# Sudaraka88/LDWeaver

Measured on NVIDIA B200. Metric: weighted SNP-pair MI/sec, higher is better.
Workload: dtype int8 (tcgen05 kind::i8 with int32 accumulation of 28-bit fixed-point weights; fp32 MI epilogue, fp64 refinement of long-range links)

## Files before the change

### ldweaver_b200/csrc/mi_aux.cuh

```cuda
#pragma once
#include "mi_types.h"

namespace ldw {

__global__ void mi_build_rec_kernel(const uint8_t* __restrict__ codes, int64_t S, const int32_t* __restrict__ slot_snp,
                                    int64_t nslots, const uint8_t* __restrict__ mask, const double* __restrict__ w,
                                    const int32_t* __restrict__ wH, const int32_t* __restrict__ wL, Rec* rec,
                                    int64_t vstride, double* p64 , uint32_t sa, uint32_t sb, uint32_t M) {
  int64_t slot = (int64_t)blockIdx.x * (blockDim.x >> 5) + (threadIdx.x >> 5);
  int lane = threadIdx.x & 31;
  if (slot >= nslots) return;
  int32_t snp = slot_snp[slot];
  if (snp < 0) {
    if (lane < 4) {
      Rec z;
      for (int q = 0; q < 4; q++) { z.T[q] = 0; z.rp[q] = 0.f; z.q[q] = 1.f; }
      z.T4 = 0; z.rp4 = 0.f; z.q4 = 1.f; z.pad = 0;
      rec[lane * vstride + slot] = z;
    }
    return;
  }
  const uint8_t* row = codes + (int64_t)snp * S;
  double p[5] = {0, 0, 0, 0, 0};
  int h[5] = {0, 0, 0, 0, 0}, l[5] = {0, 0, 0, 0, 0};
// ... 21 lines not shown
    for (int a = 0; a < 5; a++) p64[(int64_t)snp * 5 + a] = p[a];
  if (lane < 4) {
    int m = mask[snp];
    uint32_t qt[5] = {0, 0, 0, 0, 0};
    float qr[5] = {0.f, 0.f, 0.f, 0.f, 0.f}, qq[5] = {1.f, 1.f, 1.f, 1.f, 1.f};
    int q = 0;
    for (int a = 0; a < 5; a++) {
      if (m & (1 << a)) {
        qt[q] = ((uint32_t)h[a] << sa) + ((uint32_t)l[a] >> sb) + M * (uint32_t)(lane + 2);
        const double v = p[a] + 0.5 * (double)(lane + 2);
        qr[q] = (float)(1.0 / v);
        qq[q] = (float)v;
        q++;
      }
    }
    Rec z;
    for (int t = 0; t < 4; t++) { z.T[t] = qt[t]; z.rp[t] = qr[t]; z.q[t] = qq[t]; }
    z.T4 = qt[4]; z.rp4 = qr[4]; z.q4 = qq[4]; z.pad = 0;
    rec[lane * vstride + slot] = z;
  }
}

__global__ void mi_pack_operands_kernel(const uint8_t* __restrict__ codes, int64_t S, int64_t Kpad,
                                        const uint32_t* __restrict__ row_info, int64_t nrows, uint8_t* X) {
  int64_t chunks = Kpad / 16;
  int64_t id = (int64_t)blockIdx.x * blockDim.x + threadIdx.x;
  if (id >= nrows * chunks) return;
  int64_t R = id / chunks, ch = id % chunks;
  uint32_t info = row_info[R];
  uint32_t x1[4] = {0, 0, 0, 0};
  if (info != 0xFFFFFFFFu) {
    const uint8_t* row = codes + (int64_t)(info & 0x0FFFFFFF) * S;
    int al = info >> 28;
    int64_t s0 = ch * 16;
#pragma unroll
    for (int k = 0; k < 16; k++) {
      int64_t s = s0 + k;
      uint32_t bit = (s < S && row[s] == al) ? 0xFFu : 0u;
      x1[k >> 2] |= bit << (8 * (k & 3));
    }
  }
  *reinterpret_cast<uint4*>(X + R * Kpad + ch * 16) = make_uint4(x1[0], x1[1], x1[2], x1[3]);
}

struct RefineParams {
  const uint8_t* codes;
  int64_t S;
  const double* w;
  const double* p64;
  const uint8_t* r;
  const uint8_t* mask;
  const int32_t* from_idx;
  const int32_t* to_idx;
  const uint8_t* rfl_arr;
  const uint8_t* rtl_arr;
  int32_t nf, nt;
  int32_t ideal_q;
  double neff;
};

constexpr int REFINE_WARPS = 6;
__device__ __forceinline__ int heaviest_class(const double (&p)[5]) {
  int b = 0;
#pragma unroll
  for (int a = 1; a < 5; a++) b = p[a] > p[b] ? a : b;
// ... 566 lines not shown
```

### ldweaver_b200/csrc/mi_kernel.cuh

```cuda
#pragma once
#include "mi_types.h"
#include "umma.cuh"

namespace ldw {

constexpr int MI_EXP_WARPS = 6;
constexpr int MI_EXP_THREADS = 32 * MI_EXP_WARPS;
constexpr int MI_EPI_WARP0 = 8;
constexpr int MI_EPI_GROUPS = 4;
constexpr int MI_EPI_WARPS = 4 * MI_EPI_GROUPS;
constexpr int MI_EPI_THREADS = 32 * MI_EPI_WARPS;
constexpr int MI_THREADS = 32 * (MI_EPI_WARP0 + MI_EPI_WARPS);
#define LDW_STR2(x) #x
#define LDW_STR(x) LDW_STR2(x)
#define MI_REGS_CTRL 48
#define MI_REGS_EPI 96
static_assert(MI_EPI_WARP0 * 32 * MI_REGS_CTRL + MI_EPI_THREADS * MI_REGS_EPI <= MI_THREADS * ((65536 / MI_THREADS) & ~7), "register budget");
constexpr int MI_MAX_STAGES = 4;
constexpr uint32_t MI_ARR_BYTES = 128 * 128;
constexpr uint32_t MI_STAGE_REGION = 12 * MI_ARR_BYTES;
__host__ __device__ constexpr uint32_t mi_stage_need(int pa, int pb, int njlog2) {
  return (uint32_t)pa * MI_ARR_BYTES + 4u * (uint32_t)pb * (64u << njlog2);
}
__host__ __device__ constexpr int mi_stage_geo(int pa, int pb, int njlog2) {
  return mi_stage_need(pa, pb, njlog2) <= 3 * MI_ARR_BYTES ? 0 : mi_stage_need(pa, pb, njlog2) <= 4 * MI_ARR_BYTES ? 1 : 2;
}
__host__ __device__ constexpr int mi_geo_stages(int geo) { return 4 - geo; }
__host__ __device__ constexpr uint32_t mi_geo_bytes(int geo) { return geo == 0 ? 3 * MI_ARR_BYTES : geo == 1 ? 4 * MI_ARR_BYTES : 6 * MI_ARR_BYTES; }
constexpr uint32_t MI_JREC_BYTES = 128 * sizeof(Rec);
constexpr uint32_t MI_JDYN_BYTES = 128 * sizeof(ColDyn);
constexpr uint32_t MI_IREC_BYTES = 128 * sizeof(Rec);
constexpr uint32_t MI_IDYN_BYTES = 128 * sizeof(RowDyn);
constexpr uint32_t MI_BAR_BYTES = 512;
constexpr uint32_t MI_SMEM_BYTES = MI_STAGE_REGION + 2 * (MI_JREC_BYTES + MI_JDYN_BYTES) + MI_IREC_BYTES + MI_IDYN_BYTES + MI_BAR_BYTES + 1024;
static_assert(MI_SMEM_BYTES <= 232448, "shared memory budget (227 KB opt-in)");

__device__ __forceinline__ float lg2_fast(float x) {
  float y;
  asm("lg2.approx.ftz.f32 %0, %1;" : "=f"(y) : "f"(x));
  return y;
}
__device__ __forceinline__ uint32_t ld_volatile_u32(const uint32_t* p) {
  uint32_t v;
  asm volatile("ld.volatile.global.u32 %0, [%1];" : "=r"(v) : "l"(p));
  return v;
}

__host__ __device__ constexpr int mi_jc(int pa, int pb) {
  return (pa + 1) * (pb + 1) <= 4 ? 8 : (pa + 1) * (pb + 1) <= 9 ? 4 : (pa + 1) * (pb + 1) <= 12 ? 2 : 1;
}
__host__ __device__ constexpr int mi_njlog2(int pa, int pb) {
  return pa * pb == 1 ? 7 : pa * pb == 2 ? 6 : pa * pb <= 4 ? 5 : 4;
}

__device__ __noinline__ void lr_raise_threshold(const ScanParams& p, int lane) {
  constexpr int PER = MI_HIST_BINS / 32;
  uint32_t s = 0;
  for (int k = 0; k < PER; k++) s += ld_volatile_u32(p.hist + lane * PER + k);
  uint32_t suf = s;
#pragma unroll
  for (int o = 1; o < 32; o <<= 1) {
    uint32_t v = __shfl_down_sync(0xffffffffu, suf, o);
    if (lane + o < 32) suf += v;
  }
  unsigned m = __ballot_sync(0xffffffffu, suf >= p.kprime);
  if (m == 0) return;
  int sel = 31 - __clz(m);
  if (lane == sel) {
    uint32_t run = suf - s;
    for (int k = PER - 1; k >= 0; k--) {
      run += ld_volatile_u32(p.hist + lane * PER + k);
      if (run >= p.kprime) {
        atomicMax(p.tcand_bits, (uint32_t)(lane * PER + k) << 19);
        break;
      }
// ... 7 lines not shown
    long long c0 = clock64();
    mbar_wait(bar, parity, tag);
    acc += clock64() - c0;
  } else {
    mbar_wait(bar, parity, tag);
  }
}

struct EpiCtx {
  int q, cg, lane, rank;
  uint32_t tflags;
  uint32_t tmem_base;
  uint32_t jrec_saddr;
  uint32_t jdyn_saddr;
  uint32_t irec_saddr, idyn_saddr;
  uint32_t rempty_saddr;
  uint32_t scr_saddr;
};

__device__ __forceinline__ uint4 lds128(uint32_t saddr) {
  uint4 v;
  asm volatile("ld.shared.v4.u32 {%0, %1, %2, %3}, [%4];" : "=r"(v.x), "=r"(v.y), "=r"(v.z), "=r"(v.w) : "r"(saddr));
  return v;
}

__device__ __forceinline__ uint2 lds64(uint32_t saddr) {
  uint2 v;
  asm volatile("ld.shared.v2.u32 {%0, %1}, [%2];" : "=r"(v.x), "=r"(v.y) : "r"(saddr));
  return v;
}

__device__ __forceinline__ void sts128(uint32_t saddr, uint4 v) {
  asm volatile("st.shared.v4.u32 [%0], {%1, %2, %3, %4};" ::"r"(saddr), "r"(v.x), "r"(v.y), "r"(v.z), "r"(v.w) : "memory");
}

__device__ __forceinline__ float rcp_fast(float x) {
  float y;
  asm("rcp.approx.ftz.f32 %0, %1;" : "=f"(y) : "f"(x));
  return y;
}

template <bool QC>
__device__ __forceinline__ float mi_term(float acc, uint32_t t, float ra, float rb, float dq) {
  const float x = __uint2float_rn(t);
  const float ratio = QC ? x * rcp_fast(fmaf(ra, rb, dq)) : x * (ra * rb);
  return fmaf(x, lg2_fast(ratio), acc);
// ... 281 lines not shown
  switch (pa * 4 + pb - 5) {
    case 0: epi_tile<1, 1, QC, RG>(p, c, rel); break;
    case 1: epi_tile<1, 2, QC, RG>(p, c, rel); break;
    case 2: epi_tile<1, 3, QC, RG>(p, c, rel); break;
    case 3: epi_tile<1, 4, QC, RG>(p, c, rel); break;
    case 4: epi_tile<2, 1, QC, RG>(p, c, rel); break;
    case 5: epi_tile<2, 2, QC, RG>(p, c, rel); break;
    case 6: epi_tile<2, 3, QC, RG>(p, c, rel); break;
    case 7: epi_tile<2, 4, QC, RG>(p, c, rel); break;
    case 8: epi_tile<3, 1, QC, RG>(p, c, rel); break;
    case 9: epi_tile<3, 2, QC, RG>(p, c, rel); break;
    case 10: epi_tile<3, 3, QC, RG>(p, c, rel); break;
    case 11: epi_tile<3, 4, QC, RG>(p, c, rel); break;
    case 12: epi_tile<4, 1, QC, RG>(p, c, rel); break;
    case 13: epi_tile<4, 2, QC, RG>(p, c, rel); break;
    case 14: epi_tile<4, 3, QC, RG>(p, c, rel); break;
    case 15: epi_tile<4, 4, QC, RG>(p, c, rel); break;
    default: break;
  }
}

template <bool DBG>
__global__ void __cluster_dims__(2, 1, 1) __launch_bounds__(MI_THREADS, 1)
mi_scan_kernel(const __grid_constant__ TmapSet tm, const __grid_constant__ ScanParams p) {
  extern __shared__ uint8_t smem_raw[];
  uint8_t* smem = reinterpret_cast<uint8_t*>((reinterpret_cast<uintptr_t>(smem_raw) + 1023) & ~(uintptr_t)1023);
  uint8_t* stage_base = smem;
  Rec* jrec = reinterpret_cast<Rec*>(smem + MI_STAGE_REGION);
  ColDyn* jdyn = reinterpret_cast<ColDyn*>(smem + MI_STAGE_REGION + 2 * MI_JREC_BYTES);
  Rec* irec = reinterpret_cast<Rec*>(smem + MI_STAGE_REGION + 2 * (MI_JREC_BYTES + MI_JDYN_BYTES));
  RowDyn* idyn = reinterpret_cast<RowDyn*>(smem + MI_STAGE_REGION + 2 * (MI_JREC_BYTES + MI_JDYN_BYTES) + MI_IREC_BYTES);
  uint64_t* bars = reinterpret_cast<uint64_t*>(smem + MI_STAGE_REGION + 2 * (MI_JREC_BYTES + MI_JDYN_BYTES) + MI_IREC_BYTES + MI_IDYN_BYTES);
  uint64_t* full = bars;
  uint64_t* empty = bars + 4;
  uint64_t* ready = bars + 8;
  uint64_t* tfull = bars + 12;
  uint64_t* tempty = bars + 14;
  uint64_t* jfull = bars + 16;
  uint64_t* jempty = bars + 18;
  uint64_t* drained = bars + 20;
  uint64_t* rfull = bars + 21;
  uint64_t* rempty = bars + 22;
  uint32_t* tmem_slot = reinterpret_cast<uint32_t*>(bars + 23);
  uint32_t* thdr = reinterpret_cast<uint32_t*>(bars + 24);

  const int warp = threadIdx.x >> 5, lane = threadIdx.x & 31;
  const uint32_t rank = cluster_ctarank();
  if (warp == 0 && lane == 0) {
    tma_prefetch_desc(&tm.a);
    for (int i = 0; i < MI_MAX_STAGES; i++) {
      mbar_init(&full[i], 1); mbar_init(&empty[i], 1); mbar_init(&ready[i], 2 * MI_EXP_WARPS);
    }
    mbar_init(drained, 1);
    mbar_init(rfull, 1); mbar_init(rempty, MI_EPI_WARPS);
    for (int i = 0; i < 2; i++) {
      mbar_init(&tfull[i], 1); mbar_init(&tempty[i], 2 * MI_EPI_WARPS);
      mbar_init(&jfull[i], 1); mbar_init(&jempty[i], MI_EPI_WARPS);
    }
    fence_barrier_init();
  }
  if (warp == 2) tmem_alloc_pair(tmem_slot, 512);
  tc_fence_before();
  cluster_sync_all();
  tc_fence_after();
  const uint32_t tmem_base = *tmem_slot;
  const int tile0 = (int)(blockIdx.x >> 1), tstep = (int)(gridDim.x >> 1);

  if (warp < MI_EPI_WARP0) {
  asm volatile("setmaxnreg.dec.sync.aligned.u32 " LDW_STR(MI_REGS_CTRL) ";");
  if (warp == 0) {
    int st = 0; uint32_t phb = 0; int geo = -1; uint32_t dph = 0;
    int it = 0, rit = 0;
    long long w_jempty = 0, w_empty = 0, t_begin = DBG ? clock64() : 0;
    for (int t = tile0; t < p.n_tiles; t += tstep, it++) {
      const TileDesc td = p.tiles[t];
      const int PA = td.PA, PB = td.PB, NJ = 1 << td.njlog2, NJh = NJ >> 1;
      const int njidx = 7 - td.njlog2;
      const int g = mi_stage_geo(PA, PB, td.njlog2);
      const int nst = mi_geo_stages(g);
      const uint32_t sbytes = mi_geo_bytes(g);
      if (g != geo) {
        if (geo >= 0) { mbar_wait(drained, dph, 12); dph ^= 1; }
        geo = g; st = 0;
      }
      {
        const uint32_t stage_tx = (uint32_t)PA * MI_ARR_BYTES + (uint32_t)(PB * NJh * 128);
        const int a_row = td.a_row0 + (int)rank * 128, b_row = td.b_row0 + (int)rank * NJh;
        for (int kb = 0; kb < p.nkb; kb++) {
          timed_wait<DBG>(&empty[st], ((phb >> st) & 1) ^ 1, 11, w_empty);
          if (elect_one()) {
            uint8_t* sb = stage_base + st * sbytes;
            mbar_arrive_expect_tx(&full[st], stage_tx);
            for (int a = 0; a < PA; a++)
              tma_load_2d(sb + a * MI_ARR_BYTES, &tm.a, &full[st], kb * 128, a_row + a * td.a_pstride);
            uint8_t* sbB = sb + PA * MI_ARR_BYTES;
            for (int b = 0; b < PB; b++)
              tma_load_2d(sbB + b * NJh * 128, &tm.b[njidx], &full[st], kb * 128, b_row + b * td.b_pstride);
          }
          __syncwarp();
          phb ^= 1u << st;
          if (++st == nst) st = 0;
        }
      }
      const int jb = it & 1;
      timed_wait<DBG>(&jempty[jb], ((it >> 1) & 1) ^ 1, 10, w_jempty);
      if (elect_one()) {
        thdr[jb] = (uint32_t)PA | ((uint32_t)PB << 8) | ((uint32_t)td.njlog2 << 16) | ((uint32_t)(rank ? td.flags1 : td.flags) << 24);
        mbar_arrive_expect_tx(&jfull[jb], (uint32_t)NJ * (uint32_t)(sizeof(Rec) + sizeof(ColDyn)));
        bulk_load_1d(jrec + jb * 128, p.rec + (int64_t)(PA + 1 - 2) * p.rec_vstride + td.j_slot0, NJ * sizeof(Rec), &jfull[jb]);
        bulk_load_1d(jdyn + jb * 128, p.coldyn + td.j_dyn0, NJ * sizeof(ColDyn), &jfull[jb]);
      }
      __syncwarp();
      if (!((rank ? td.flags1 : td.flags) & TILE_NULL)) {
        timed_wait<DBG>(rempty, (uint32_t)(rit & 1) ^ 1, 13, w_jempty);
        if (elect_one()) {
          mbar_arrive_expect_tx(rfull, MI_IREC_BYTES + MI_IDYN_BYTES);
          bulk_load_1d(irec, p.rec + (int64_t)(PB + 1 - 2) * p.rec_vstride + td.i_slot0 + (int)rank * 128, MI_IREC_BYTES, rfull);
          bulk_load_1d(idyn, p.rowdyn + td.i_dyn0 + (int)rank * 128, MI_IDYN_BYTES, rfull);
        }
        __syncwarp();
        rit++;
      }
    }
    if (DBG && p.dbg && lane == 0) {
// ... 65 lines not shown
      }
      if (elect_one()) {
        if (sw) umma_commit_pair(drained);
        if (big) {
          umma_commit_pair(&tfull[0]);
          umma_commit_pair(&tfull[1]);
        } else {
          umma_commit_pair(&tfull[as]);
        }
      }
      __syncwarp();
      if (!big) {
        if (++as == 2) { as = 0; aph ^= 1; }
      }
    }
    if (DBG && p.dbg && lane == 0) {
      p.dbg[blockIdx.x * 16 + 3] = (unsigned long long)(clock64() - t_begin);
      p.dbg[blockIdx.x * 16 + 4] = (unsigned long long)w_tempty;
      p.dbg[blockIdx.x * 16 + 5] = (unsigned long long)w_ready;
    }
    }
  } else {
    const int h = (warp - 2) * 32 + lane;
    int st = 0; uint32_t phb = 0; int geo = -1;
    long long w_full = 0, t_begin = DBG ? clock64() : 0;
    for (int t = tile0; t < p.n_tiles; t += tstep) {
      const TileDesc td = p.tiles[t];
      const int PA = td.PA, PB = td.PB, NJh = (1 << td.njlog2) >> 1;
      const int brows = PB * NJh;
      const int g = mi_stage_geo(PA, PB, td.njlog2);
      const int nst = mi_geo_stages(g);
      const uint32_t sbytes = mi_geo_bytes(g);
      if (g != geo) { geo = g; st = 0; }
      for (int kb = 0; kb < p.nkb; kb++) {
        const int cl = h & 7;
        const uint8_t* dg = p.dig + (int64_t)kb * 128 + cl * 16;
        const uint4 g0 = __ldg(reinterpret_cast<const uint4*>(dg));
        const uint4 g1 = __ldg(reinterpret_cast<const uint4*>(dg + p.kpad));
        const uint4 g2 = __ldg(reinterpret_cast<const uint4*>(dg + 2 * p.kpad));
        const uint4 g3 = __ldg(reinterpret_cast<const uint4*>(dg + 3 * p.kpad));
        timed_wait<DBG>(&full[st], (phb >> st) & 1, 40, w_full);
        const uint32_t yb = smem_u32(stage_base + st * sbytes) + (uint32_t)PA * MI_ARR_BYTES;
        const uint32_t slot = (uint32_t)brows * 128u;
        for (int r = h >> 3; r < brows; r += MI_EXP_THREADS / 8) {
          const uint32_t addr = yb + (uint32_t)r * 128u + (uint32_t)((cl ^ (r & 7)) * 16);
          const uint4 y = lds128(addr);
          sts128(addr + slot, make_uint4(y.x & g1.x, y.y & g1.y, y.z & g1.z, y.w & g1.w));
          sts128(addr + 2 * slot, make_uint4(y.x & g2.x, y.y & g2.y, y.z & g2.z, y.w & g2.w));
          sts128(addr + 3 * slot, make_uint4(y.x & g3.x, y.y & g3.y, y.z & g3.z, y.w & g3.w));
          sts128(addr, make_uint4(y.x & g0.x, y.y & g0.y, y.z & g0.z, y.w & g0.w));
        }
        fence_proxy_async_smem();
        __syncwarp();
        if (lane == 0) mbar_arrive_cluster(&ready[st], 0);
        phb ^= 1u << st;
        if (++st == nst) st = 0;
      }
    }
    if (DBG && p.dbg && h == 0) {
      p.dbg[blockIdx.x * 16 + 12] = (unsigned long long)(clock64() - t_begin);
      p.dbg[blockIdx.x * 16 + 13] = (unsigned long long)w_full;
    }
  }
  } else {
    asm volatile("setmaxnreg.inc.sync.aligned.u32 " LDW_STR(MI_REGS_EPI) ";");
    EpiCtx c;
    c.q = warp & 3;
    c.cg = (warp - MI_EPI_WARP0) >> 2;
    c.lane = lane;
    c.rank = (int)rank;
    int as = 0; uint32_t aph = 0;
    int it = 0, rit = 0;
    long long w_jfull = 0, w_tfull = 0, t_begin = DBG ? clock64() : 0;
    c.irec_saddr = smem_u32(irec);
    c.idyn_saddr = smem_u32(idyn);
    c.rempty_saddr = smem_u32(rempty);
    c.scr_saddr = smem_u32(bars + 32) + (uint32_t)(warp - MI_EPI_WARP0) * 4u;
    for (int t = tile0; t < p.n_tiles; t += tstep, it++) {
      const int jb = it & 1;
      timed_wait<DBG>(&jfull[jb], (it >> 1) & 1, 30, w_jfull);
      uint32_t hdr;
      asm volatile("ld.shared.u32 %0, [%1];" : "=r"(hdr) : "r"(smem_u32(&thdr[jb])));
      const int tPA = (int)(hdr & 0xFF), tPB = (int)((hdr >> 8) & 0xFF);
      c.tflags = hdr >> 24;
// ... 58 lines not shown
```

### ldweaver_b200/csrc/mi_scan.cu

```cuda
#include <algorithm>
#include <chrono>
#include <cmath>
#include <cub/cub.cuh>
#include <vector>

#include "../../include/ldw.h"
#include "ctx.h"
#include "hdw.h"
#include "mi_aux.cuh"
#include "mi_kernel.cuh"
#include "mi_scan.h"

using namespace ldw;

namespace {

struct Group {
  int32_t slot0 = 0, nslots = 0, row0 = 0, count = 0;
};

struct DevLinks {
  DevBuf pos1, pos2, c1, c2, len, blk, mi;
  int ensure(int64_t m) {
    size_t b4 = (size_t)(m > 0 ? m : 1) * 4, b8 = (size_t)(m > 0 ? m : 1) * 8;
// ... 56 lines not shown
};

static void scan_ws_free(void* p) { delete static_cast<ScanWS*>(p); }

static ScanWS* get_ws(ldw_ctx* ctx) {
  if (!ctx->scan_ws) {
    ctx->scan_ws = new ScanWS();
    ctx->scan_ws_free = scan_ws_free;
  }
  return static_cast<ScanWS*>(ctx->scan_ws);
}

struct ldw_mi_plan {
  ldw_ctx* ctx = nullptr;
  int64_t n = 0, S = 0, blk = 0, Kpad = 0;
  int nranges = 0;
  std::vector<int32_t> pos, paint;
  std::vector<uint8_t> r, mask;
  std::vector<double> w;
  std::vector<Group> groups;
  std::vector<int32_t> range_slot0;
  std::vector<int32_t> slot_snp;
  int64_t nslots = 0, nrows = 0;
  double neff = 0, scale = 0;
  int32_t neffH = 0, neffL = 0;
  uint32_t sa = 0, sb = 0;
  uint32_t M = 0;
  bool pos_sorted = true;
  DevBuf d_codes, d_w, d_p64, d_rec, d_r, d_mask, d_pos, d_paint, d_ops, d_dig;
  const uint8_t* codes_dev = nullptr;
  TmapSet tm;
  std::vector<BlockResult> results;
  double t_pack_ms = 0;
};

namespace {

int build_plan(ldw_mi_plan* P, const uint8_t* codes, const uint8_t* codes_dev, const double* hdw, const int32_t* pos,
               const int32_t* paint) {
  ldw_ctx* ctx = P->ctx;
  cudaStream_t st = ctx->stream;
  const int64_t n = P->n, S = P->S, blk = P->blk;
  cudaEvent_t e0, e1;
  LDW_CUDA(cudaEventCreate(&e0));
  LDW_CUDA(cudaEventCreate(&e1));
  LDW_CUDA(cudaEventRecord(e0, st));
  const bool dbg_t = getenv("LDW_DBG_TIMING") != nullptr;
  auto bt0 = std::chrono::steady_clock::now();
  auto blap = [&](const char* what) {
    if (!dbg_t) return;
    auto t = std::chrono::steady_clock::now();
    fprintf(stderr, "ldw timing: plan %-22s %8.3f ms\n", what, std::chrono::duration<double, std::milli>(t - bt0).count());
    bt0 = t;
  };
// ... 144 lines not shown
  LDW_TRY(P->d_w.alloc((size_t)S * 8));
  LDW_TRY(d_wH.alloc((size_t)S * 4));
  LDW_TRY(d_wL.alloc((size_t)S * 4));
  LDW_TRY(d_slot_snp.alloc((size_t)std::max<int64_t>(slot, 1) * 4));
  LDW_TRY(d_row_info.alloc(row_info.size() * 4));
  LDW_TRY(P->d_p64.alloc((size_t)n * 5 * 8));
  LDW_TRY(P->d_rec.alloc((size_t)std::max<int64_t>(slot, 1) * 4 * sizeof(Rec)));
  LDW_TRY(P->d_pos.alloc((size_t)n * 4));
  LDW_TRY(P->d_paint.alloc((size_t)n * 4));
  LDW_CUDA(cudaMemcpyAsync(P->d_w.p, hdw, (size_t)S * 8, cudaMemcpyHostToDevice, st));
  LDW_CUDA(cudaMemcpyAsync(d_wH.p, wH.data(), (size_t)S * 4, cudaMemcpyHostToDevice, st));
  LDW_CUDA(cudaMemcpyAsync(d_wL.p, wL.data(), (size_t)S * 4, cudaMemcpyHostToDevice, st));
  LDW_CUDA(cudaMemcpyAsync(d_slot_snp.p, P->slot_snp.data(), (size_t)slot * 4, cudaMemcpyHostToDevice, st));
  LDW_CUDA(cudaMemcpyAsync(d_row_info.p, row_info.data(), row_info.size() * 4, cudaMemcpyHostToDevice, st));
  LDW_CUDA(cudaMemcpyAsync(P->d_pos.p, pos, (size_t)n * 4, cudaMemcpyHostToDevice, st));
  LDW_CUDA(cudaMemcpyAsync(P->d_paint.p, paint, (size_t)n * 4, cudaMemcpyHostToDevice, st));
  {
    int wpb = 8;
    mi_build_rec_kernel<<<(unsigned)((slot + wpb - 1) / wpb), wpb * 32, 0, st>>>(
        P->codes_dev, S, d_slot_snp.as<int32_t>(), slot, P->d_mask.as<uint8_t>(), P->d_w.as<double>(),
        d_wH.as<int32_t>(), d_wL.as<int32_t>(), P->d_rec.as<Rec>(), slot, P->d_p64.as<double>(), P->sa, P->sb, P->M);
    LDW_CUDA(cudaGetLastError());
  }
  size_t op_bytes = (size_t)std::max<int64_t>(row, 128) * P->Kpad;
  LDW_TRY(P->d_ops.alloc(op_bytes));
  LDW_TRY(P->d_dig.alloc(dig.size()));
  LDW_CUDA(cudaMemcpyAsync(P->d_dig.p, dig.data(), dig.size(), cudaMemcpyHostToDevice, st));
  {
    int64_t total = row * (P->Kpad / 16);
    if (total > 0) {
      mi_pack_operands_kernel<<<(unsigned)((total + 255) / 256), 256, 0, st>>>(P->codes_dev, S, P->Kpad,
                                                                               d_row_info.as<uint32_t>(), row,
                                                                               P->d_ops.as<uint8_t>());
      LDW_CUDA(cudaGetLastError());
    }
  }
  uint64_t trows = (uint64_t)std::max<int64_t>(row, 128);
  LDW_TRY(make_tmap_u8_sw128(&P->tm.a, P->d_ops.p, trows, (uint64_t)P->Kpad, 128));
  for (int j = 0; j < 4; j++) LDW_TRY(make_tmap_u8_sw128(&P->tm.b[j], P->d_ops.p, trows, (uint64_t)P->Kpad, 64u >> j));
  {
    ScanWS* W = get_ws(ctx);
    if (!W->events_ready) {
      for (auto& b : W->ring) {
        LDW_CUDA(cudaEventCreateWithFlags(&b.done, cudaEventDisableTiming));
        LDW_CUDA(cudaEventCreateWithFlags(&b.done2, cudaEventDisableTiming));
        LDW_CUDA(cudaEventCreateWithFlags(&b.uploaded, cudaEventDisableTiming));
      }
      for (auto& l : W->lr) {
        LDW_CUDA(cudaEventCreateWithFlags(&l.scan_done, cudaEventDisableTiming));
        LDW_CUDA(cudaEventCreateWithFlags(&l.sel_done, cudaEventDisableTiming));
      }
      W->events_ready = true;
    }
  }
  LDW_CUDA(cudaEventRecord(e1, st));
  LDW_CUDA(cudaStreamSynchronize(st));
  blap("records + pack + tmaps");
  float ms = 0;
  cudaEventElapsedTime(&ms, e0, e1);
  P->t_pack_ms = ms;
  cudaEventDestroy(e0);
  cudaEventDestroy(e1);
  LDW_CUDA(cudaFuncSetAttribute(mi_scan_kernel<false>, cudaFuncAttributeMaxDynamicSharedMemorySize, MI_SMEM_BYTES));
  LDW_CUDA(cudaFuncSetAttribute(mi_scan_kernel<true>, cudaFuncAttributeMaxDynamicSharedMemorySize, MI_SMEM_BYTES));
  return 0;
}

struct ScanCfg {
  double g, sr_dist, lr_retain, lr_approx;
  int flags;
  int dense = 0;
};

inline double circ_len_d(double p1, double p2, double g) {
  double m = std::fmod(p1 - p2, g);
  if (m < 0) m += g;
  return 0.5 * g - std::fabs(m - 0.5 * g);
}

int prepare_block(const ldw_mi_plan* P, int bf, int bt, const ScanCfg& cfg, BlockHost& H, bool sizes_only = false) {
// ... 233 lines not shown
      memcpy(D.stage.as<uint8_t>() + off, p.src, p.bytes);
      LDW_CUDA(cudaMemcpyAsync(p.d->p, D.stage.as<uint8_t>() + off, p.bytes, cudaMemcpyHostToDevice, st));
    }
    off += (p.bytes + 255) & ~(size_t)255;
  }
  return 0;
}

void fill_scan_params(const ldw_mi_plan* P, const BlockDev& D, const BlockHost& H, const ScanCfg& cfg, ScanParams& sp) {
  memset(&sp, 0, sizeof(sp));
  sp.tiles = D.tiles.as<TileDesc>();
  sp.n_tiles = H.n_real_tiles;
  sp.rec = P->d_rec.as<Rec>();
  sp.rec_vstride = P->nslots;
  sp.rowdyn = D.rowdyn.as<RowDyn>();
  sp.coldyn = D.coldyn.as<ColDyn>();
  sp.nkb = (int32_t)(P->Kpad / 128);
  sp.nf = H.nf; sp.nt = H.nt;
  sp.diag = H.diag; sp.ragged = H.ragged;
  sp.qcorr = (!H.diag && !(cfg.flags & LDW_SCAN_IDEAL_Q)) ? 1 : 0;
  sp.sr_only = (cfg.flags & LDW_SCAN_SR_ONLY) ? 1 : 0;
  sp.dig = P->d_dig.as<uint8_t>();
  sp.kpad = P->Kpad;
  sp.rfl_arr = D.rfl.as<uint8_t>();
  sp.rtl_arr = D.rtl.as<uint8_t>();
  sp.sa = P->sa;
  sp.sb = P->sb;
  sp.kT = (float)(std::ldexp(1.0, (int)P->sb) / P->scale);
  sp.M = P->M;
  for (int a = 0; a < 4; a++)
    for (int b = 0; b < 4; b++) {
      double ri = a + 2, rj = b + 2;
      double den = P->neff + 0.5 * ri * rj;
      const float den_f = (float)den, rkT = 1.0f / sp.kT, rden = 1.0f / den_f;
      sp.scale[a][b] = (float)(M_LN2 / den) * sp.kT;
      sp.q0s[a][b] = (float)(0.25 * ri * rj / den) * rkT;
      sp.qod[a][b] = (float)(0.25 / den) * rkT;
      sp.rp_qc[a][b] = rden * rkT;
      sp.rp_plain[a][b] = den_f * sp.kT;
    }
}

int launch_scan(const ldw_mi_plan* P, const ScanParams& sp, cudaStream_t st, int reserve = 0) {
  if (sp.n_tiles <= 0) return 0;
  int grid = 2 * std::min<int>(sp.n_tiles, std::max(1, (P->ctx->num_sms - reserve) / 2));
  if (sp.dbg) mi_scan_kernel<true><<<grid, MI_THREADS, MI_SMEM_BYTES, st>>>(P->tm, sp);
  else mi_scan_kernel<false><<<grid, MI_THREADS, MI_SMEM_BYTES, st>>>(P->tm, sp);
  LDW_CUDA(cudaGetLastError());
  return 0;
}

RefineParams make_refine_params(const ldw_mi_plan* P, const BlockDev& D, const BlockHost& H, const ScanCfg& cfg) {
  RefineParams R;
  R.codes = P->codes_dev;
  R.S = P->S;
  R.w = P->d_w.as<double>();
  R.p64 = P->d_p64.as<double>();
  R.r = P->d_r.as<uint8_t>();
  R.mask = P->d_mask.as<uint8_t>();
  R.from_idx = D.from_idx.as<int32_t>();
  R.to_idx = D.to_idx.as<int32_t>();
  R.rfl_arr = D.rfl.as<uint8_t>();
  R.rtl_arr = D.rtl.as<uint8_t>();
  R.nf = H.nf; R.nt = H.nt;
  R.ideal_q = (cfg.flags & LDW_SCAN_IDEAL_Q) ? 1 : 0;
  R.neff = P->neff;
  return R;
}

int validate_scan(const ldw_mi_plan* P, const ScanCfg& cfg) {
// ... 719 lines not shown
    }
    stats_out->n_scan_launches = n_scan_launches;
    stats_out->n_launches = n_launches;
    stats_out->n_tiles = n_tiles;
    stats_out->exec_int8_ops = exec_ops;
    stats_out->t_host_prep_ms = host_prep_ms;
    stats_out->exec_mufu_ops = exec_mufu;
    {
      double em = 0;
      for (size_t b = 0; b < blocks.size(); b++)
        if (!sel[b].skip && sel[b].n_lr > 0 && !sr_only) em = std::max(em, (double)P->results[b].eps_obs);
      stats_out->eps_obs_max = em;
    }
  }
  if (dbg_block >= 0 && W->d_dbg.p) {
    std::vector<unsigned long long> h(4096 * 16);
    cudaMemcpy(h.data(), W->d_dbg.p, h.size() * 8, cudaMemcpyDeviceToHost);
    double s[16] = {0};
    int nb = 0;
    for (int c = 0; c < 4096; c++)
      if (h[c * 16 + 3]) { nb++; for (int k = 0; k < 16; k++) s[k] += (double)h[c * 16 + k]; }
    if (nb) {
      fprintf(stderr, "ldw dbg block %lld (%d CTAs, kilo-cycles avg): producer total %.0f wait_jempty %.0f wait_empty %.0f | "
              "mma total %.0f wait_tempty %.0f wait_ready %.0f | expander total %.0f wait_full %.0f | epi(first) total %.0f "
              "wait_jfull %.0f wait_tfull %.0f | epi(last) total %.0f wait_jfull %.0f wait_tfull %.0f\n", (long long)dbg_block, nb,
              s[0] / nb / 1e3, s[1] / nb / 1e3, s[2] / nb / 1e3, s[3] / nb / 1e3, s[4] / nb / 1e3, s[5] / nb / 1e3, s[12] / nb / 1e3,
              s[13] / nb / 1e3, s[6] / nb / 1e3, s[7] / nb / 1e3, s[8] / nb / 1e3, s[9] / nb / 1e3, s[10] / nb / 1e3, s[11] / nb / 1e3);
    }
  }
  kev_cleanup();
  cudaEventDestroy(ev0); cudaEventDestroy(ev1); cudaEventDestroy(ev2); cudaEventDestroy(ev3);
  lap("borderline + stats (host)");
  return 0;
}
```

### ldweaver_b200/csrc/mi_types.h

```cpp
#pragma once
#include <cuda.h>
#include <stdint.h>

namespace ldw {

struct __align__(16) Rec {
  uint32_t T[4];
  float rp[4];
  float q[4];
  uint32_t T4;
  float rp4;
  float q4;
  uint32_t pad;
};
static_assert(sizeof(Rec) == 64, "Rec must be 64 bytes");

struct RowDyn {
  int32_t il;
  float rtl;
};

struct __align__(16) ColDyn {
  int32_t jl;
  float rfl;
// ... 33 lines not shown
  int32_t nf, nt;
  int32_t diag, ragged, qcorr, sr_only, dense, emit_all;
  const uint8_t* rfl_arr;
  const uint8_t* rtl_arr;
  float kT;
  uint32_t sa, sb;
  uint32_t M;
  float scale[4][4];
  float q0s[4][4];
  float qod[4][4];
  float rp_qc[4][4];
  float rp_plain[4][4];
  float* sr_out;
  float* dense_out;
  Cand* cand;
  uint32_t cand_cap;
  uint32_t* cand_count;
  uint32_t* tcand_bits;
  uint32_t* hist;
  uint32_t kprime, delta;
  uint32_t* overflow;
  const uint8_t* dig;
  int64_t kpad;
  unsigned long long* dbg;
};

struct TmapSet {
  CUtensorMap a;
  CUtensorMap b[4];
};

}
```

Measured before the change: 85.81 billion.

## Stream bit-packed operands and expand to int8 in shared memory

Operands are now stored in global memory as 1-bit-per-sample packed words in a k-block-major layout instead of one byte per sample. They are bulk-copied into a small packed ring in shared memory. The expander warps turn them into swizzled 0/0xFF int8 tiles with prmt, which replaces the TMA 2D loads and tensor maps. The aim is to cut global/L2 operand traffic by about 8x in exchange for more expander work, a new two-level barrier pipeline, and fewer, differently sized stage geometries.

```diff
diff --git a/ldweaver_b200/csrc/mi_aux.cuh b/ldweaver_b200/csrc/mi_aux.cuh
--- a/ldweaver_b200/csrc/mi_aux.cuh
+++ b/ldweaver_b200/csrc/mi_aux.cuh
@@ -67,25 +67,24 @@
 }
 
 __global__ void mi_pack_operands_kernel(const uint8_t* __restrict__ codes, int64_t S, int64_t Kpad,
-                                        const uint32_t* __restrict__ row_info, int64_t nrows, uint8_t* X) {
-  int64_t chunks = Kpad / 16;
-  int64_t id = (int64_t)blockIdx.x * blockDim.x + threadIdx.x;
-  if (id >= nrows * chunks) return;
-  int64_t R = id / chunks, ch = id % chunks;
-  uint32_t info = row_info[R];
-  uint32_t x1[4] = {0, 0, 0, 0};
+                                        const uint32_t* __restrict__ row_info, int64_t nrows, int64_t xrows, uint32_t* Xp) {
+  const int64_t id = (int64_t)blockIdx.x * blockDim.x + threadIdx.x;
+  if (id >= (Kpad / 128) * xrows * 4) return;
+  const int64_t kb = id / (xrows * 4), R = (id / 4) % xrows;
+  const int w = (int)(id & 3);
+  const uint32_t info = R < nrows ? row_info[R] : 0xFFFFFFFFu;
+  uint32_t x = 0;
   if (info != 0xFFFFFFFFu) {
     const uint8_t* row = codes + (int64_t)(info & 0x0FFFFFFF) * S;
-    int al = info >> 28;
-    int64_t s0 = ch * 16;
-#pragma unroll
-    for (int k = 0; k < 16; k++) {
-      int64_t s = s0 + k;
-      uint32_t bit = (s < S && row[s] == al) ? 0xFFu : 0u;
-      x1[k >> 2] |= bit << (8 * (k & 3));
-    }
-  }
-  *reinterpret_cast<uint4*>(X + R * Kpad + ch * 16) = make_uint4(x1[0], x1[1], x1[2], x1[3]);
+    const uint8_t al = (uint8_t)(info >> 28);
+    const int64_t s0 = kb * 128 + w * 32;
+#pragma unroll 8
+    for (int k = 0; k < 32; k++) {
+      const int64_t s = s0 + k;
+      if (s < S && row[s] == al) x |= 1u << (8 * (k & 3) + (k >> 2));
+    }
+  }
+  Xp[id] = x;
 }
 
 struct RefineParams {
diff --git a/ldweaver_b200/csrc/mi_kernel.cuh b/ldweaver_b200/csrc/mi_kernel.cuh
--- a/ldweaver_b200/csrc/mi_kernel.cuh
+++ b/ldweaver_b200/csrc/mi_kernel.cuh
@@ -16,17 +16,34 @@
 #define MI_REGS_CTRL 48
 #define MI_REGS_EPI 96
 static_assert(MI_EPI_WARP0 * 32 * MI_REGS_CTRL + MI_EPI_THREADS * MI_REGS_EPI <= MI_THREADS * ((65536 / MI_THREADS) & ~7), "register budget");
-constexpr int MI_MAX_STAGES = 4;
 constexpr uint32_t MI_ARR_BYTES = 128 * 128;
+__host__ __device__ constexpr int mi_njlog2(int pa, int pb) {
+  return pa * pb == 1 ? 7 : pa * pb == 2 ? 6 : pa * pb <= 4 ? 5 : 4;
+}
 constexpr uint32_t MI_STAGE_REGION = 12 * MI_ARR_BYTES;
+constexpr uint32_t MI_PK_REGION = 24 * 1024;
+constexpr uint32_t MI_EXP_REGION = MI_STAGE_REGION - MI_PK_REGION;
+constexpr int MI_MAX_STAGES = 3;
+constexpr int MI_MAX_PK = 8;
 __host__ __device__ constexpr uint32_t mi_stage_need(int pa, int pb, int njlog2) {
   return (uint32_t)pa * MI_ARR_BYTES + 4u * (uint32_t)pb * (64u << njlog2);
 }
 __host__ __device__ constexpr int mi_stage_geo(int pa, int pb, int njlog2) {
-  return mi_stage_need(pa, pb, njlog2) <= 3 * MI_ARR_BYTES ? 0 : mi_stage_need(pa, pb, njlog2) <= 4 * MI_ARR_BYTES ? 1 : 2;
-}
-__host__ __device__ constexpr int mi_geo_stages(int geo) { return 4 - geo; }
-__host__ __device__ constexpr uint32_t mi_geo_bytes(int geo) { return geo == 0 ? 3 * MI_ARR_BYTES : geo == 1 ? 4 * MI_ARR_BYTES : 6 * MI_ARR_BYTES; }
+  return mi_stage_need(pa, pb, njlog2) <= 56 * 1024 ? 0 : 1;
+}
+__host__ __device__ constexpr int mi_geo_stages(int geo) { return 3 - geo; }
+__host__ __device__ constexpr uint32_t mi_geo_bytes(int geo) { return geo == 0 ? 56 * 1024 : 80 * 1024; }
+static_assert(mi_geo_stages(0) * mi_geo_bytes(0) <= MI_EXP_REGION && mi_geo_stages(1) * mi_geo_bytes(1) <= MI_EXP_REGION &&
+              mi_stage_need(4, 4, mi_njlog2(4, 4)) <= mi_geo_bytes(1) && mi_stage_need(4, 1, mi_njlog2(4, 1)) <= mi_geo_bytes(1),
+              "stage geometries");
+__host__ __device__ constexpr uint32_t mi_pk_bytes(int pa, int pb, int njlog2) {
+  return 16u * (uint32_t)(pa * 128 + pb * ((1 << njlog2) >> 1));
+}
+__host__ __device__ constexpr int mi_pk_slots(uint32_t pk_bytes) {
+  return MI_PK_REGION / pk_bytes < (uint32_t)MI_MAX_PK ? (int)(MI_PK_REGION / pk_bytes) : MI_MAX_PK;
+}
+static_assert(mi_pk_slots(mi_pk_bytes(4, 4, mi_njlog2(4, 4))) >= 2 && mi_pk_slots(mi_pk_bytes(4, 1, mi_njlog2(4, 1))) >= 2,
+              "packed ring");
 constexpr uint32_t MI_JREC_BYTES = 128 * sizeof(Rec);
 constexpr uint32_t MI_JDYN_BYTES = 128 * sizeof(ColDyn);
 constexpr uint32_t MI_IREC_BYTES = 128 * sizeof(Rec);
@@ -48,9 +65,6 @@
 
 __host__ __device__ constexpr int mi_jc(int pa, int pb) {
   return (pa + 1) * (pb + 1) <= 4 ? 8 : (pa + 1) * (pb + 1) <= 9 ? 4 : (pa + 1) * (pb + 1) <= 12 ? 2 : 1;
-}
-__host__ __device__ constexpr int mi_njlog2(int pa, int pb) {
-  return pa * pb == 1 ? 7 : pa * pb == 2 ? 6 : pa * pb <= 4 ? 5 : 4;
 }
 
 __device__ __noinline__ void lr_raise_threshold(const ScanParams& p, int lane) {
@@ -104,6 +118,18 @@
   uint4 v;
   asm volatile("ld.shared.v4.u32 {%0, %1, %2, %3}, [%4];" : "=r"(v.x), "=r"(v.y), "=r"(v.z), "=r"(v.w) : "r"(saddr));
   return v;
+}
+
+__device__ __forceinline__ uint32_t lds32(uint32_t saddr) {
+  uint32_t v;
+  asm volatile("ld.shared.u32 %0, [%1];" : "=r"(v) : "r"(saddr));
+  return v;
+}
+
+__device__ __forceinline__ uint32_t mi_expand4(uint32_t xs) {
+  uint32_t y;
+  asm("prmt.b32 %0, %1, 0, 0xBA98;" : "=r"(y) : "r"(xs));
+  return y;
 }
 
 __device__ __forceinline__ uint2 lds64(uint32_t saddr) {
@@ -431,18 +457,20 @@
 
 template <bool DBG>
 __global__ void __cluster_dims__(2, 1, 1) __launch_bounds__(MI_THREADS, 1)
-mi_scan_kernel(const __grid_constant__ TmapSet tm, const __grid_constant__ ScanParams p) {
+mi_scan_kernel(const __grid_constant__ ScanParams p) {
   extern __shared__ uint8_t smem_raw[];
   uint8_t* smem = reinterpret_cast<uint8_t*>((reinterpret_cast<uintptr_t>(smem_raw) + 1023) & ~(uintptr_t)1023);
   uint8_t* stage_base = smem;
+  uint8_t* pk_base = smem + MI_EXP_REGION;
   Rec* jrec = reinterpret_cast<Rec*>(smem + MI_STAGE_REGION);
   ColDyn* jdyn = reinterpret_cast<ColDyn*>(smem + MI_STAGE_REGION + 2 * MI_JREC_BYTES);
   Rec* irec = reinterpret_cast<Rec*>(smem + MI_STAGE_REGION + 2 * (MI_JREC_BYTES + MI_JDYN_BYTES));
   RowDyn* idyn = reinterpret_cast<RowDyn*>(smem + MI_STAGE_REGION + 2 * (MI_JREC_BYTES + MI_JDYN_BYTES) + MI_IREC_BYTES);
   uint64_t* bars = reinterpret_cast<uint64_t*>(smem + MI_STAGE_REGION + 2 * (MI_JREC_BYTES + MI_JDYN_BYTES) + MI_IREC_BYTES + MI_IDYN_BYTES);
-  uint64_t* full = bars;
-  uint64_t* empty = bars + 4;
-  uint64_t* ready = bars + 8;
+  uint64_t* empty = bars;
+  uint64_t* ready = bars + 4;
+  uint64_t* pfull = bars + 40;
+  uint64_t* pempty = bars + 48;
   uint64_t* tfull = bars + 12;
   uint64_t* tempty = bars + 14;
   uint64_t* jfull = bars + 16;
@@ -456,9 +484,11 @@
   const int warp = threadIdx.x >> 5, lane = threadIdx.x & 31;
   const uint32_t rank = cluster_ctarank();
   if (warp == 0 && lane == 0) {
-    tma_prefetch_desc(&tm.a);
     for (int i = 0; i < MI_MAX_STAGES; i++) {
-      mbar_init(&full[i], 1); mbar_init(&empty[i], 1); mbar_init(&ready[i], 2 * MI_EXP_WARPS);
+      mbar_init(&empty[i], 1); mbar_init(&ready[i], 2 * MI_EXP_WARPS);
+    }
+    for (int i = 0; i < MI_MAX_PK; i++) {
+      mbar_init(&pfull[i], 1); mbar_init(&pempty[i], MI_EXP_WARPS);
     }
     mbar_init(drained, 1);
     mbar_init(rfull, 1); mbar_init(rempty, MI_EPI_WARPS);
@@ -478,37 +508,33 @@
   if (warp < MI_EPI_WARP0) {
   asm volatile("setmaxnreg.dec.sync.aligned.u32 " LDW_STR(MI_REGS_CTRL) ";");
   if (warp == 0) {
-    int st = 0; uint32_t phb = 0; int geo = -1; uint32_t dph = 0;
+    int ps = 0, npk = 0; uint32_t pph = 0, pkb = 0;
     int it = 0, rit = 0;
     long long w_jempty = 0, w_empty = 0, t_begin = DBG ? clock64() : 0;
     for (int t = tile0; t < p.n_tiles; t += tstep, it++) {
       const TileDesc td = p.tiles[t];
       const int PA = td.PA, PB = td.PB, NJ = 1 << td.njlog2, NJh = NJ >> 1;
-      const int njidx = 7 - td.njlog2;
-      const int g = mi_stage_geo(PA, PB, td.njlog2);
-      const int nst = mi_geo_stages(g);
-      const uint32_t sbytes = mi_geo_bytes(g);
-      if (g != geo) {
-        if (geo >= 0) { mbar_wait(drained, dph, 12); dph ^= 1; }
-        geo = g; st = 0;
+      const uint32_t kpkb = mi_pk_bytes(PA, PB, td.njlog2);
+      if (kpkb != pkb) {
+        for (int i = 0; i < npk; i++) timed_wait<DBG>(&pempty[i], ((pph >> i) & 1) ^ 1, 11, w_empty);
+        pkb = kpkb; npk = mi_pk_slots(pkb); ps = 0;
       }
       {
-        const uint32_t stage_tx = (uint32_t)PA * MI_ARR_BYTES + (uint32_t)(PB * NJh * 128);
         const int a_row = td.a_row0 + (int)rank * 128, b_row = td.b_row0 + (int)rank * NJh;
         for (int kb = 0; kb < p.nkb; kb++) {
-          timed_wait<DBG>(&empty[st], ((phb >> st) & 1) ^ 1, 11, w_empty);
+          timed_wait<DBG>(&pempty[ps], ((pph >> ps) & 1) ^ 1, 11, w_empty);
           if (elect_one()) {
-            uint8_t* sb = stage_base + st * sbytes;
-            mbar_arrive_expect_tx(&full[st], stage_tx);
+            uint8_t* dst = pk_base + ps * pkb;
+            const uint8_t* src = p.xpk + (int64_t)kb * p.xrows * 16;
+            mbar_arrive_expect_tx(&pfull[ps], pkb);
             for (int a = 0; a < PA; a++)
-              tma_load_2d(sb + a * MI_ARR_BYTES, &tm.a, &full[st], kb * 128, a_row + a * td.a_pstride);
-            uint8_t* sbB = sb + PA * MI_ARR_BYTES;
+              bulk_load_1d(dst + a * 2048, src + (int64_t)(a_row + a * td.a_pstride) * 16, 2048, &pfull[ps]);
             for (int b = 0; b < PB; b++)
-              tma_load_2d(sbB + b * NJh * 128, &tm.b[njidx], &full[st], kb * 128, b_row + b * td.b_pstride);
+              bulk_load_1d(dst + PA * 2048 + b * NJh * 16, src + (int64_t)(b_row + b * td.b_pstride) * 16, NJh * 16, &pfull[ps]);
           }
           __syncwarp();
-          phb ^= 1u << st;
-          if (++st == nst) st = 0;
+          pph ^= 1u << ps;
+          if (++ps == npk) ps = 0;
         }
       }
       const int jb = it & 1;
@@ -620,44 +646,78 @@
     }
   } else {
     const int h = (warp - 2) * 32 + lane;
-    int st = 0; uint32_t phb = 0; int geo = -1;
-    long long w_full = 0, t_begin = DBG ? clock64() : 0;
+    const int cl = h & 7;
+    const uint32_t sh = 4u - 4u * (uint32_t)(cl & 1);
+    int st = 0, geo = -1, ps = 0, npk = 0; uint32_t ph = 0, pkb = 0;
+    long long w_full = 0, w_empty = 0, t_begin = DBG ? clock64() : 0;
     for (int t = tile0; t < p.n_tiles; t += tstep) {
       const TileDesc td = p.tiles[t];
       const int PA = td.PA, PB = td.PB, NJh = (1 << td.njlog2) >> 1;
-      const int brows = PB * NJh;
+      const int arows = PA * 128, rows = arows + PB * NJh;
+      const uint32_t slot = (uint32_t)(PB * NJh) * 128u;
       const int g = mi_stage_geo(PA, PB, td.njlog2);
       const int nst = mi_geo_stages(g);
       const uint32_t sbytes = mi_geo_bytes(g);
-      if (g != geo) { geo = g; st = 0; }
+      if (g != geo) {
+        if (geo >= 0) { timed_wait<DBG>(drained, (ph >> 16) & 1, 12, w_empty); ph ^= 1u << 16; }
+        geo = g; st = 0;
+      }
+      const uint32_t kpkb = mi_pk_bytes(PA, PB, td.njlog2);
+      if (kpkb != pkb) { pkb = kpkb; npk = mi_pk_slots(pkb); ps = 0; }
       for (int kb = 0; kb < p.nkb; kb++) {
-        const int cl = h & 7;
-        const uint8_t* dg = p.dig + (int64_t)kb * 128 + cl * 16;
-        const uint4 g0 = __ldg(reinterpret_cast<const uint4*>(dg));
-        const uint4 g1 = __ldg(reinterpret_cast<const uint4*>(dg + p.kpad));
-        const uint4 g2 = __ldg(reinterpret_cast<const uint4*>(dg + 2 * p.kpad));
-        const uint4 g3 = __ldg(reinterpret_cast<const uint4*>(dg + 3 * p.kpad));
-        timed_wait<DBG>(&full[st], (phb >> st) & 1, 40, w_full);
-        const uint32_t yb = smem_u32(stage_base + st * sbytes) + (uint32_t)PA * MI_ARR_BYTES;
-        const uint32_t slot = (uint32_t)brows * 128u;
-        for (int r = h >> 3; r < brows; r += MI_EXP_THREADS / 8) {
-          const uint32_t addr = yb + (uint32_t)r * 128u + (uint32_t)((cl ^ (r & 7)) * 16);
-          const uint4 y = lds128(addr);
-          sts128(addr + slot, make_uint4(y.x & g1.x, y.y & g1.y, y.z & g1.z, y.w & g1.w));
-          sts128(addr + 2 * slot, make_uint4(y.x & g2.x, y.y & g2.y, y.z & g2.z, y.w & g2.w));
-          sts128(addr + 3 * slot, make_uint4(y.x & g3.x, y.y & g3.y, y.z & g3.z, y.w & g3.w));
-          sts128(addr, make_uint4(y.x & g0.x, y.y & g0.y, y.z & g0.z, y.w & g0.w));
+        timed_wait<DBG>(&pfull[ps], (ph >> (8 + ps)) & 1, 40, w_full);
+        timed_wait<DBG>(&empty[st], ((ph >> st) & 1) ^ 1, 41, w_empty);
+        const uint32_t xb = smem_u32(pk_base + ps * pkb) + (uint32_t)(cl >> 1) * 4u;
+        const uint32_t yb = smem_u32(stage_base + st * sbytes) + (uint32_t)cl * 16u;
+        int r = h >> 3;
+        constexpr int RS = MI_EXP_THREADS / 8;
+        for (; r + 3 * RS < arows; r += 4 * RS) {
+          uint32_t x[4];
+#pragma unroll
+          for (int u = 0; u < 4; u++) x[u] = lds32(xb + (uint32_t)(r + u * RS) * 16u) << sh;
+#pragma unroll
+          for (int u = 0; u < 4; u++) {
+            const int ru = r + u * RS;
+            sts128((yb ^ (uint32_t)((ru & 7) * 16)) + (uint32_t)ru * 128u,
+                   make_uint4(mi_expand4(x[u] << 3), mi_expand4(x[u] << 2), mi_expand4(x[u] << 1), mi_expand4(x[u])));
+          }
+        }
+        for (; r < arows; r += MI_EXP_THREADS / 8) {
+          const uint32_t x = lds32(xb + (uint32_t)r * 16u) << sh;
+          sts128((yb ^ (uint32_t)((r & 7) * 16)) + (uint32_t)r * 128u,
+                 make_uint4(mi_expand4(x << 3), mi_expand4(x << 2), mi_expand4(x << 1), mi_expand4(x)));
+        }
+        if (r < rows) {
+          const uint8_t* dg = p.dig + (int64_t)kb * 128 + cl * 16;
+          const uint4 g0 = __ldg(reinterpret_cast<const uint4*>(dg));
+          const uint4 g1 = __ldg(reinterpret_cast<const uint4*>(dg + p.kpad));
+          const uint4 g2 = __ldg(reinterpret_cast<const uint4*>(dg + 2 * p.kpad));
+          const uint4 g3 = __ldg(reinterpret_cast<const uint4*>(dg + 3 * p.kpad));
+          for (; r < rows; r += MI_EXP_THREADS / 8) {
+            const uint32_t x = lds32(xb + (uint32_t)r * 16u) << sh;
+            const uint4 y = make_uint4(mi_expand4(x << 3), mi_expand4(x << 2), mi_expand4(x << 1), mi_expand4(x));
+            const uint32_t addr = (yb ^ (uint32_t)((r & 7) * 16)) + (uint32_t)r * 128u;
+            sts128(addr, make_uint4(y.x & g0.x, y.y & g0.y, y.z & g0.z, y.w & g0.w));
+            sts128(addr + slot, make_uint4(y.x & g1.x, y.y & g1.y, y.z & g1.z, y.w & g1.w));
+            sts128(addr + 2 * slot, make_uint4(y.x & g2.x, y.y & g2.y, y.z & g2.z, y.w & g2.w));
+            sts128(addr + 3 * slot, make_uint4(y.x & g3.x, y.y & g3.y, y.z & g3.z, y.w & g3.w));
+          }
         }
         fence_proxy_async_smem();
         __syncwarp();
-        if (lane == 0) mbar_arrive_cluster(&ready[st], 0);
-        phb ^= 1u << st;
+        if (lane == 0) {
+          mbar_arrive(&pempty[ps]);
+          mbar_arrive_cluster(&ready[st], 0);
+        }
+        ph ^= (1u << st) | (256u << ps);
         if (++st == nst) st = 0;
+        if (++ps == npk) ps = 0;
       }
     }
     if (DBG && p.dbg && h == 0) {
       p.dbg[blockIdx.x * 16 + 12] = (unsigned long long)(clock64() - t_begin);
       p.dbg[blockIdx.x * 16 + 13] = (unsigned long long)w_full;
+      p.dbg[blockIdx.x * 16 + 14] = (unsigned long long)w_empty;
     }
   }
   } else {
diff --git a/ldweaver_b200/csrc/mi_scan.cu b/ldweaver_b200/csrc/mi_scan.cu
--- a/ldweaver_b200/csrc/mi_scan.cu
+++ b/ldweaver_b200/csrc/mi_scan.cu
@@ -102,6 +102,7 @@
   std::vector<int32_t> range_slot0;
   std::vector<int32_t> slot_snp;
   int64_t nslots = 0, nrows = 0;
+  int64_t xrows = 0;
   double neff = 0, scale = 0;
   int32_t neffH = 0, neffL = 0;
   uint32_t sa = 0, sb = 0;
@@ -109,7 +110,6 @@
   bool pos_sorted = true;
   DevBuf d_codes, d_w, d_p64, d_rec, d_r, d_mask, d_pos, d_paint, d_ops, d_dig;
   const uint8_t* codes_dev = nullptr;
-  TmapSet tm;
   std::vector<BlockResult> results;
   double t_pack_ms = 0;
 };
@@ -300,22 +300,17 @@
         d_wH.as<int32_t>(), d_wL.as<int32_t>(), P->d_rec.as<Rec>(), slot, P->d_p64.as<double>(), P->sa, P->sb, P->M);
     LDW_CUDA(cudaGetLastError());
   }
-  size_t op_bytes = (size_t)std::max<int64_t>(row, 128) * P->Kpad;
-  LDW_TRY(P->d_ops.alloc(op_bytes));
+  P->xrows = row + 128;
+  LDW_TRY(P->d_ops.alloc((size_t)P->xrows * (size_t)(P->Kpad / 8)));
   LDW_TRY(P->d_dig.alloc(dig.size()));
   LDW_CUDA(cudaMemcpyAsync(P->d_dig.p, dig.data(), dig.size(), cudaMemcpyHostToDevice, st));
   {
-    int64_t total = row * (P->Kpad / 16);
-    if (total > 0) {
-      mi_pack_operands_kernel<<<(unsigned)((total + 255) / 256), 256, 0, st>>>(P->codes_dev, S, P->Kpad,
-                                                                               d_row_info.as<uint32_t>(), row,
-                                                                               P->d_ops.as<uint8_t>());
-      LDW_CUDA(cudaGetLastError());
-    }
-  }
-  uint64_t trows = (uint64_t)std::max<int64_t>(row, 128);
-  LDW_TRY(make_tmap_u8_sw128(&P->tm.a, P->d_ops.p, trows, (uint64_t)P->Kpad, 128));
-  for (int j = 0; j < 4; j++) LDW_TRY(make_tmap_u8_sw128(&P->tm.b[j], P->d_ops.p, trows, (uint64_t)P->Kpad, 64u >> j));
+    const int64_t words = (P->Kpad / 128) * P->xrows * 4;
+    mi_pack_operands_kernel<<<(unsigned)((words + 255) / 256), 256, 0, st>>>(P->codes_dev, S, P->Kpad,
+                                                                             d_row_info.as<uint32_t>(), row, P->xrows,
+                                                                             P->d_ops.as<uint32_t>());
+    LDW_CUDA(cudaGetLastError());
+  }
   {
     ScanWS* W = get_ws(ctx);
     if (!W->events_ready) {
@@ -333,7 +328,7 @@
   }
   LDW_CUDA(cudaEventRecord(e1, st));
   LDW_CUDA(cudaStreamSynchronize(st));
-  blap("records + pack + tmaps");
+  blap("records + pack");
   float ms = 0;
   cudaEventElapsedTime(&ms, e0, e1);
   P->t_pack_ms = ms;
@@ -613,6 +608,8 @@
   sp.sr_only = (cfg.flags & LDW_SCAN_SR_ONLY) ? 1 : 0;
   sp.dig = P->d_dig.as<uint8_t>();
   sp.kpad = P->Kpad;
+  sp.xpk = P->d_ops.as<uint8_t>();
+  sp.xrows = P->xrows;
   sp.rfl_arr = D.rfl.as<uint8_t>();
   sp.rtl_arr = D.rtl.as<uint8_t>();
   sp.sa = P->sa;
@@ -635,8 +632,8 @@
 int launch_scan(const ldw_mi_plan* P, const ScanParams& sp, cudaStream_t st, int reserve = 0) {
   if (sp.n_tiles <= 0) return 0;
   int grid = 2 * std::min<int>(sp.n_tiles, std::max(1, (P->ctx->num_sms - reserve) / 2));
-  if (sp.dbg) mi_scan_kernel<true><<<grid, MI_THREADS, MI_SMEM_BYTES, st>>>(P->tm, sp);
-  else mi_scan_kernel<false><<<grid, MI_THREADS, MI_SMEM_BYTES, st>>>(P->tm, sp);
+  if (sp.dbg) mi_scan_kernel<true><<<grid, MI_THREADS, MI_SMEM_BYTES, st>>>(sp);
+  else mi_scan_kernel<false><<<grid, MI_THREADS, MI_SMEM_BYTES, st>>>(sp);
   LDW_CUDA(cudaGetLastError());
   return 0;
 }
@@ -1402,10 +1399,10 @@
       if (h[c * 16 + 3]) { nb++; for (int k = 0; k < 16; k++) s[k] += (double)h[c * 16 + k]; }
     if (nb) {
       fprintf(stderr, "ldw dbg block %lld (%d CTAs, kilo-cycles avg): producer total %.0f wait_jempty %.0f wait_empty %.0f | "
-              "mma total %.0f wait_tempty %.0f wait_ready %.0f | expander total %.0f wait_full %.0f | epi(first) total %.0f "
+              "mma total %.0f wait_tempty %.0f wait_ready %.0f | expander total %.0f wait_full %.0f wait_empty %.0f | epi(first) total %.0f "
               "wait_jfull %.0f wait_tfull %.0f | epi(last) total %.0f wait_jfull %.0f wait_tfull %.0f\n", (long long)dbg_block, nb,
               s[0] / nb / 1e3, s[1] / nb / 1e3, s[2] / nb / 1e3, s[3] / nb / 1e3, s[4] / nb / 1e3, s[5] / nb / 1e3, s[12] / nb / 1e3,
-              s[13] / nb / 1e3, s[6] / nb / 1e3, s[7] / nb / 1e3, s[8] / nb / 1e3, s[9] / nb / 1e3, s[10] / nb / 1e3, s[11] / nb / 1e3);
+              s[13] / nb / 1e3, s[14] / nb / 1e3, s[6] / nb / 1e3, s[7] / nb / 1e3, s[8] / nb / 1e3, s[9] / nb / 1e3, s[10] / nb / 1e3, s[11] / nb / 1e3);
     }
   }
   kev_cleanup();
diff --git a/ldweaver_b200/csrc/mi_types.h b/ldweaver_b200/csrc/mi_types.h
--- a/ldweaver_b200/csrc/mi_types.h
+++ b/ldweaver_b200/csrc/mi_types.h
@@ -79,12 +79,9 @@
   uint32_t* overflow;
   const uint8_t* dig;
   int64_t kpad;
+  const uint8_t* xpk;
+  int64_t xrows;
   unsigned long long* dbg;
 };
 
-struct TmapSet {
-  CUtensorMap a;
-  CUtensorMap b[4];
-};
-
 }
```

Result: slower. 65.08 billion, median of 6 (-24.2%).
